# caiyuanhao1998/Open-DiffusionGS

Hardware: NVIDIA H100
Metric: denoise_steps_per_sec (higher is better)
Workload: dtype bf16

## Files before the change

### open-diffusiongs_b200/csrc/attention_sm90.cu

```cuda
#include "dgs_internal.h"
#include "dit_kernels.h"
#include "sm90_ptx.cuh"

namespace dgs {

using namespace ptx;

constexpr int ATT_BM = 128, ATT_BN = 128, ATT_HD = 64, ATT_KV_STAGES = 3, ATT_THREADS = WS_THREADS;
constexpr int ATT_Q_BYTES = ATT_BM * ATT_HD * 2;
constexpr int ATT_KV_BYTES = ATT_BN * ATT_HD * 2;
constexpr int ATT_SMEM_BYTES = ATT_Q_BYTES + 2 * ATT_KV_STAGES * ATT_KV_BYTES + 1024 + 256;

__global__ void __launch_bounds__(ATT_THREADS, 1)
attention_fwd_kernel(const __grid_constant__ CUtensorMap tm_qkv, __nv_bfloat16* __restrict__ out, float* __restrict__ lse2,
                     int Np, int N, int H) {
  extern __shared__ uint8_t smem_raw[];
  const uint32_t raw = smem_u32(smem_raw);
  uint8_t* smem = smem_raw + (((raw + 1023u) & ~1023u) - raw);
  uint8_t* sQ = smem;
  uint8_t* sK = sQ + ATT_Q_BYTES;
  uint8_t* sV = sK + ATT_KV_STAGES * ATT_KV_BYTES;
  uint64_t* q_full = reinterpret_cast<uint64_t*>(sV + ATT_KV_STAGES * ATT_KV_BYTES);
  uint64_t* k_full = q_full + 1;
  uint64_t* v_full = k_full + ATT_KV_STAGES;
  uint64_t* kv_empty = v_full + ATT_KV_STAGES;

  const int warp = threadIdx.x >> 5, lane = threadIdx.x & 31;
  const int q0 = blockIdx.x * ATT_BM, h = blockIdx.y, b = blockIdx.z;
  const int n_blocks = (N + ATT_BN - 1) / ATT_BN;
  const int D = H * ATT_HD;

  if (threadIdx.x == 0) {
    prefetch_tmap(&tm_qkv);
    mbar_init(q_full, 1);
    for (int s = 0; s < ATT_KV_STAGES; s++) { mbar_init(k_full + s, 1); mbar_init(v_full + s, 1); mbar_init(kv_empty + s, 8); }
    fence_barrier_init();
  }
  __syncthreads();
  griddep_launch_dependents();
  griddep_wait();

  if (warp >= 8) {
    ws_producer_regs();
    if (warp == 8 && lane == 0) {
      mbar_arrive_expect_tx(q_full, ATT_Q_BYTES);
      tma_load_3d(sQ, &tm_qkv, q_full, h * ATT_HD, q0, b);
      for (int j = 0; j < n_blocks; j++) {
        const int s = j % ATT_KV_STAGES;
        mbar_wait(kv_empty + s, ((uint32_t)(j / ATT_KV_STAGES) & 1) ^ 1);
        mbar_arrive_expect_tx(k_full + s, ATT_KV_BYTES);
        tma_load_3d(sK + s * ATT_KV_BYTES, &tm_qkv, k_full + s, D + h * ATT_HD, j * ATT_BN, b);
        mbar_arrive_expect_tx(v_full + s, ATT_KV_BYTES);
        tma_load_3d(sV + s * ATT_KV_BYTES, &tm_qkv, v_full + s, 2 * D + h * ATT_HD, j * ATT_BN, b);
      }
    }
    return;
  }

  ws_consumer_regs();
  const int wg = warp >> 2;
  const int quad_col = 2 * (lane & 3);
  const int r0 = wg * 64 + (warp & 3) * 16 + (lane >> 2);
  const float sl2 = 0.125f * 1.4426950408889634f;
  const uint64_t qdesc = wg_desc_sw128(smem_u32(sQ + wg * 8192), 16, 1024);
  float o[32];
#pragma unroll
  for (int i = 0; i < 32; i++) o[i] = 0.f;
  float m_run[2] = {-INFINITY, -INFINITY}, l_run[2] = {0.f, 0.f};
  mbar_wait(q_full, 0);
  for (int j = 0; j < n_blocks; j++) {
    const int s = j % ATT_KV_STAGES;
    const uint32_t use = (uint32_t)(j / ATT_KV_STAGES) & 1;
    float sc[64];
#pragma unroll
    for (int i = 0; i < 64; i++) sc[i] = 0.f;
    mbar_wait(k_full + s, use);
    {
      const uint64_t kdesc = wg_desc_sw128(smem_u32(sK + s * ATT_KV_BYTES), 16, 1024);
      wg_fence();
#pragma unroll
      for (int k = 0; k < ATT_HD / 16; k++) wgmma_m64n128_ss<0, 0>(sc, qdesc + (uint64_t)(2 * k), kdesc + (uint64_t)(2 * k));
      wg_commit();
      wg_wait<0>();
      wg_fence_regs(sc);
    }
    const int kv_valid = N - j * ATT_BN;
    if (kv_valid < ATT_BN) {
#pragma unroll
      for (int jj = 0; jj < 16; jj++)
#pragma unroll
        for (int e = 0; e < 4; e++)
          if (8 * jj + quad_col + (e & 1) >= kv_valid) sc[4 * jj + e] = -INFINITY;
    }
    float alpha[2], moff[2];
#pragma unroll
    for (int i = 0; i < 2; i++) {
      float mx = -INFINITY;
#pragma unroll
      for (int jj = 0; jj < 16; jj++) mx = fmaxf(mx, fmaxf(sc[4 * jj + 2 * i], sc[4 * jj + 2 * i + 1]));
      mx = fmaxf(mx, __shfl_xor_sync(0xffffffffu, mx, 1));
      mx = fmaxf(mx, __shfl_xor_sync(0xffffffffu, mx, 2));
      const float m_new = fmaxf(m_run[i], mx);
      alpha[i] = ex2_approx((m_run[i] - m_new) * sl2);
      m_run[i] = m_new;
      moff[i] = m_new * sl2;
    }
    uint32_t pa[8][4];
    float ls[2] = {0.f, 0.f};
#pragma unroll
    for (int kk = 0; kk < 8; kk++) {
#pragma unroll
      for (int q = 0; q < 4; q++) {
        const int idx = 8 * kk + 4 * (q >> 1) + 2 * (q & 1);
        const float p0 = ex2_approx(fmaf(sc[idx], sl2, -moff[q & 1]));
        const float p1 = ex2_approx(fmaf(sc[idx + 1], sl2, -moff[q & 1]));
        ls[q & 1] += p0 + p1;
        pa[kk][q] = pack2_bf16(p0, p1);
      }
    }
#pragma unroll
    for (int i = 0; i < 2; i++) l_run[i] = l_run[i] * alpha[i] + ls[i];
#pragma unroll
    for (int jj = 0; jj < 8; jj++) {
      o[4 * jj + 0] *= alpha[0]; o[4 * jj + 1] *= alpha[0];
      o[4 * jj + 2] *= alpha[1]; o[4 * jj + 3] *= alpha[1];
    }
    mbar_wait(v_full + s, use);
    {
      const uint64_t vdesc = wg_desc_sw128(smem_u32(sV + s * ATT_KV_BYTES), 8192, 1024);
      wg_fence();
#pragma unroll
      for (int kk = 0; kk < 8; kk++) wgmma_m64n64_rs<1>(o, pa[kk], vdesc + (uint64_t)(128 * kk));
      wg_commit();
      wg_wait<0>();
      wg_fence_regs(o);
    }
    __syncwarp();
    if (lane == 0) mbar_arrive(kv_empty + s);
  }
#pragma unroll
  for (int i = 0; i < 2; i++) {
    l_run[i] += __shfl_xor_sync(0xffffffffu, l_run[i], 1);
    l_run[i] += __shfl_xor_sync(0xffffffffu, l_run[i], 2);
  }
#pragma unroll
  for (int i = 0; i < 2; i++) {
    const int q = q0 + r0 + 8 * i;
    if (q >= N) continue;
    if (lse2 && (lane & 3) == 0) lse2[((size_t)b * H + h) * Np + q] = fmaf(m_run[i], sl2, log2f(l_run[i]));
    const float inv = 1.0f / l_run[i];
    __nv_bfloat16* dst = out + ((size_t)b * N + q) * D + h * ATT_HD + quad_col;
#pragma unroll
    for (int jj = 0; jj < 8; jj++)
      *reinterpret_cast<uint32_t*>(dst + 8 * jj) = pack2_bf16(o[4 * jj + 2 * i] * inv, o[4 * jj + 2 * i + 1] * inv);
  }
}

int attention_fwd(const void* qkv, void* out, float* lse2, int B, int N, int H, cudaStream_t st) {
  DGS_REQUIRE(B > 0 && N > 0 && H > 0, "attention: bad shape B=%d N=%d H=%d", B, N, H);
  const int D = H * ATT_HD;
  const int Np = attention_lse_stride(N);
  CUtensorMap tm_qkv;
  uint64_t dims[3] = {(uint64_t)(3 * D), (uint64_t)N, (uint64_t)B};
  uint64_t str[2] = {(uint64_t)(3 * D) * 2, (uint64_t)N * 3 * D * 2};
  uint32_t box[3] = {ATT_HD, ATT_BM, 1};
  int rc = make_tmap_bf16(&tm_qkv, qkv, 3, dims, str, box);
  if (rc) return rc;
  static bool configured = false;
  if (!configured) {
    DGS_CUDA_OK(cudaFuncSetAttribute(attention_fwd_kernel, cudaFuncAttributeMaxDynamicSharedMemorySize, ATT_SMEM_BYTES));
    configured = true;
  }
  dim3 grid(ceil_div(N, ATT_BM), H, B);
  DGS_CUDA_OK(launch_pdl(attention_fwd_kernel, grid, dim3(ATT_THREADS), ATT_SMEM_BYTES, st, tm_qkv,
                         reinterpret_cast<__nv_bfloat16*>(out), lse2, Np, N, H));
  DGS_POST_LAUNCH();
  return DGS_OK;
}

}
```

### open-diffusiongs_b200/csrc/sm90_ptx.cuh

```cuda
#pragma once
#include <cuda.h>
#include <cuda_bf16.h>
#include <cuda_runtime.h>

#include <cstdint>

namespace dgs {
namespace ptx {

__device__ __forceinline__ uint32_t smem_u32(const void* p) { return (uint32_t)__cvta_generic_to_shared(p); }

__device__ __forceinline__ void mbar_init(uint64_t* bar, uint32_t count) {
  asm volatile("mbarrier.init.shared::cta.b64 [%0], %1;" ::"r"(smem_u32(bar)), "r"(count) : "memory");
}
__device__ __forceinline__ void fence_barrier_init() { asm volatile("fence.mbarrier_init.release.cluster;" ::: "memory"); }
__device__ __forceinline__ void fence_proxy_async() { asm volatile("fence.proxy.async.shared::cta;" ::: "memory"); }
__device__ __forceinline__ void mbar_arrive_expect_tx(uint64_t* bar, uint32_t bytes) {
  asm volatile("mbarrier.arrive.expect_tx.shared::cta.b64 _, [%0], %1;" ::"r"(smem_u32(bar)), "r"(bytes) : "memory");
}
__device__ __forceinline__ void mbar_arrive(uint64_t* bar) {
  asm volatile("mbarrier.arrive.shared::cta.b64 _, [%0];" ::"r"(smem_u32(bar)) : "memory");
}
__device__ __forceinline__ bool mbar_try_wait(uint64_t* bar, uint32_t parity) {
  uint32_t ok;
  asm volatile(
      "{\n\t.reg .pred p;\n\t"
      "mbarrier.try_wait.parity.shared::cta.b64 p, [%1], %2;\n\t"
      "selp.b32 %0, 1, 0, p;\n\t}"
      : "=r"(ok)
      : "r"(smem_u32(bar)), "r"(parity)
      : "memory");
  return ok != 0;
}
__device__ __forceinline__ bool mbar_try_wait_hint(uint64_t* bar, uint32_t parity, uint32_t hint_ns) {
  uint32_t ok;
  asm volatile(
      "{\n\t.reg .pred p;\n\t"
      "mbarrier.try_wait.parity.shared::cta.b64 p, [%1], %2, %3;\n\t"
      "selp.b32 %0, 1, 0, p;\n\t}"
      : "=r"(ok)
      : "r"(smem_u32(bar)), "r"(parity), "r"(hint_ns)
      : "memory");
  return ok != 0;
}
#ifndef DGS_MBAR_TIMEOUT_SPINS
#define DGS_MBAR_TIMEOUT_SPINS 200000u
#endif
__device__ __forceinline__ void mbar_wait(uint64_t* bar, uint32_t parity) {
  if (mbar_try_wait(bar, parity)) return;
  uint32_t spins = 0;
  while (!mbar_try_wait_hint(bar, parity, 20000u)) {
    if (++spins > DGS_MBAR_TIMEOUT_SPINS) __trap();
  }
}

constexpr int WS_THREADS = 384;
__device__ __forceinline__ void ws_producer_regs() { asm volatile("setmaxnreg.dec.sync.aligned.u32 40;"); }
__device__ __forceinline__ void ws_consumer_regs() { asm volatile("setmaxnreg.inc.sync.aligned.u32 232;"); }

__device__ __forceinline__ void griddep_wait() { asm volatile("griddepcontrol.wait;" ::: "memory"); }
__device__ __forceinline__ void griddep_launch_dependents() { asm volatile("griddepcontrol.launch_dependents;" ::: "memory"); }

__device__ __forceinline__ void prefetch_tmap(const CUtensorMap* m) {
  asm volatile("prefetch.tensormap [%0];" ::"l"(reinterpret_cast<uint64_t>(m)) : "memory");
}
__device__ __forceinline__ void tma_load_2d(void* smem_dst, const CUtensorMap* m, uint64_t* bar, int c0, int c1) {
  asm volatile(
      "cp.async.bulk.tensor.2d.shared::cluster.global.mbarrier::complete_tx::bytes [%0], [%1, {%3, %4}], [%2];" ::"r"(
          smem_u32(smem_dst)),
      "l"(reinterpret_cast<uint64_t>(m)), "r"(smem_u32(bar)), "r"(c0), "r"(c1)
      : "memory");
}
__device__ __forceinline__ void tma_load_3d(void* smem_dst, const CUtensorMap* m, uint64_t* bar, int c0, int c1, int c2) {
  asm volatile(
      "cp.async.bulk.tensor.3d.shared::cluster.global.mbarrier::complete_tx::bytes [%0], [%1, {%3, %4, %5}], [%2];" ::"r"(
          smem_u32(smem_dst)),
      "l"(reinterpret_cast<uint64_t>(m)), "r"(smem_u32(bar)), "r"(c0), "r"(c1), "r"(c2)
      : "memory");
}
__device__ __forceinline__ void tma_store_2d(const CUtensorMap* m, const void* smem_src, int c0, int c1) {
  asm volatile("cp.async.bulk.tensor.2d.global.shared::cta.bulk_group [%0, {%2, %3}], [%1];" ::"l"(
                   reinterpret_cast<uint64_t>(m)),
               "r"(smem_u32(smem_src)), "r"(c0), "r"(c1)
               : "memory");
}
__device__ __forceinline__ void tma_reduce_add_2d(const CUtensorMap* m, const void* smem_src, int c0, int c1) {
  asm volatile("cp.reduce.async.bulk.tensor.2d.global.shared::cta.add.tile.bulk_group [%0, {%2, %3}], [%1];" ::"l"(
                   reinterpret_cast<uint64_t>(m)),
               "r"(smem_u32(smem_src)), "r"(c0), "r"(c1)
               : "memory");
}
__device__ __forceinline__ void bulk_commit() { asm volatile("cp.async.bulk.commit_group;" ::: "memory"); }
template <int N>
__device__ __forceinline__ void bulk_wait_read() { asm volatile("cp.async.bulk.wait_group.read %0;" ::"n"(N) : "memory"); }
template <int N>
__device__ __forceinline__ void bulk_wait() { asm volatile("cp.async.bulk.wait_group %0;" ::"n"(N) : "memory"); }
__device__ __forceinline__ void named_bar_sync(int id, int threads) {
  asm volatile("bar.sync %0, %1;" ::"r"(id), "r"(threads) : "memory");
}

__device__ __forceinline__ float ex2_approx(float x) {
  float y;
  asm("ex2.approx.ftz.f32 %0, %1;" : "=f"(y) : "f"(x));
  return y;
}
__device__ __forceinline__ uint32_t pack2_bf16(float a, float b) {
  __nv_bfloat162 v = __floats2bfloat162_rn(a, b);
  return *reinterpret_cast<uint32_t*>(&v);
}

__device__ __forceinline__ uint64_t wg_desc_sw128(uint32_t smem_addr, uint32_t lbo_bytes, uint32_t sbo_bytes) {
  uint64_t d = 0;
  d |= (uint64_t)((smem_addr & 0x3FFFFu) >> 4);
  d |= (uint64_t)((lbo_bytes >> 4) & 0x3FFFu) << 16;
  d |= (uint64_t)((sbo_bytes >> 4) & 0x3FFFu) << 32;
  d |= (uint64_t)1 << 62;
  return d;
}
__device__ __forceinline__ void wg_fence() { asm volatile("wgmma.fence.sync.aligned;" ::: "memory"); }
__device__ __forceinline__ void wg_commit() { asm volatile("wgmma.commit_group.sync.aligned;" ::: "memory"); }
template <int N>
__device__ __forceinline__ void wg_wait() { asm volatile("wgmma.wait_group.sync.aligned %0;" ::"n"(N) : "memory"); }
template <int R>
__device__ __forceinline__ void wg_fence_regs(float (&d)[R]) {
#pragma unroll
  for (int i = 0; i < R; i++) asm volatile("" : "+f"(d[i])::"memory");
}

template <int TA, int TB>
__device__ __forceinline__ void wgmma_m64n256_ss(float (&d)[128], uint64_t da, uint64_t db) {
  asm volatile(
      "wgmma.mma_async.sync.aligned.m64n256k16.f32.bf16.bf16 "
      "{%0, %1, %2, %3, %4, %5, %6, %7, %8, %9, %10, %11, %12, %13, %14, %15, %16, %17, %18, %19, %20, %21, %22, %23, %24, %25, %26, %27, %28, %29, %30, %31, %32, %33, %34, %35, %36, %37, %38, %39, %40, %41, %42, %43, %44, %45, %46, %47, %48, %49, %50, %51, %52, %53, %54, %55, %56, %57, %58, %59, %60, %61, %62, %63, %64, %65, %66, %67, %68, %69, %70, %71, %72, %73, %74, %75, %76, %77, %78, %79, %80, %81, %82, %83, %84, %85, %86, %87, %88, %89, %90, %91, %92, %93, %94, %95, %96, %97, %98, %99, %100, %101, %102, %103, %104, %105, %106, %107, %108, %109, %110, %111, %112, %113, %114, %115, %116, %117, %118, %119, %120, %121, %122, %123, %124, %125, %126, %127}, %128, %129, 1, 1, 1, %130, %131;"
      : "+f"(d[0]), "+f"(d[1]), "+f"(d[2]), "+f"(d[3]), "+f"(d[4]), "+f"(d[5]), "+f"(d[6]), "+f"(d[7]), "+f"(d[8]), "+f"(d[9]), "+f"(d[10]), "+f"(d[11]), "+f"(d[12]), "+f"(d[13]), "+f"(d[14]), "+f"(d[15]), "+f"(d[16]), "+f"(d[17]), "+f"(d[18]), "+f"(d[19]), "+f"(d[20]), "+f"(d[21]), "+f"(d[22]), "+f"(d[23]), "+f"(d[24]), "+f"(d[25]), "+f"(d[26]), "+f"(d[27]), "+f"(d[28]), "+f"(d[29]), "+f"(d[30]), "+f"(d[31]), "+f"(d[32]), "+f"(d[33]), "+f"(d[34]), "+f"(d[35]), "+f"(d[36]), "+f"(d[37]), "+f"(d[38]), "+f"(d[39]), "+f"(d[40]), "+f"(d[41]), "+f"(d[42]), "+f"(d[43]), "+f"(d[44]), "+f"(d[45]), "+f"(d[46]), "+f"(d[47]), "+f"(d[48]), "+f"(d[49]), "+f"(d[50]), "+f"(d[51]), "+f"(d[52]), "+f"(d[53]), "+f"(d[54]), "+f"(d[55]), "+f"(d[56]), "+f"(d[57]), "+f"(d[58]), "+f"(d[59]), "+f"(d[60]), "+f"(d[61]), "+f"(d[62]), "+f"(d[63]), "+f"(d[64]), "+f"(d[65]), "+f"(d[66]), "+f"(d[67]), "+f"(d[68]), "+f"(d[69]), "+f"(d[70]), "+f"(d[71]), "+f"(d[72]), "+f"(d[73]), "+f"(d[74]), "+f"(d[75]), "+f"(d[76]), "+f"(d[77]), "+f"(d[78]), "+f"(d[79]), "+f"(d[80]), "+f"(d[81]), "+f"(d[82]), "+f"(d[83]), "+f"(d[84]), "+f"(d[85]), "+f"(d[86]), "+f"(d[87]), "+f"(d[88]), "+f"(d[89]), "+f"(d[90]), "+f"(d[91]), "+f"(d[92]), "+f"(d[93]), "+f"(d[94]), "+f"(d[95]), "+f"(d[96]), "+f"(d[97]), "+f"(d[98]), "+f"(d[99]), "+f"(d[100]), "+f"(d[101]), "+f"(d[102]), "+f"(d[103]), "+f"(d[104]), "+f"(d[105]), "+f"(d[106]), "+f"(d[107]), "+f"(d[108]), "+f"(d[109]), "+f"(d[110]), "+f"(d[111]), "+f"(d[112]), "+f"(d[113]), "+f"(d[114]), "+f"(d[115]), "+f"(d[116]), "+f"(d[117]), "+f"(d[118]), "+f"(d[119]), "+f"(d[120]), "+f"(d[121]), "+f"(d[122]), "+f"(d[123]), "+f"(d[124]), "+f"(d[125]), "+f"(d[126]), "+f"(d[127])
      : "l"(da), "l"(db), "n"(TA), "n"(TB));
}
template <int TA, int TB>
__device__ __forceinline__ void wgmma_m64n128_ss(float (&d)[64], uint64_t da, uint64_t db) {
  asm volatile(
      "wgmma.mma_async.sync.aligned.m64n128k16.f32.bf16.bf16 "
      "{%0, %1, %2, %3, %4, %5, %6, %7, %8, %9, %10, %11, %12, %13, %14, %15, %16, %17, %18, %19, %20, %21, %22, %23, %24, %25, %26, %27, %28, %29, %30, %31, %32, %33, %34, %35, %36, %37, %38, %39, %40, %41, %42, %43, %44, %45, %46, %47, %48, %49, %50, %51, %52, %53, %54, %55, %56, %57, %58, %59, %60, %61, %62, %63}, %64, %65, 1, 1, 1, %66, %67;"
      : "+f"(d[0]), "+f"(d[1]), "+f"(d[2]), "+f"(d[3]), "+f"(d[4]), "+f"(d[5]), "+f"(d[6]), "+f"(d[7]), "+f"(d[8]), "+f"(d[9]), "+f"(d[10]), "+f"(d[11]), "+f"(d[12]), "+f"(d[13]), "+f"(d[14]), "+f"(d[15]), "+f"(d[16]), "+f"(d[17]), "+f"(d[18]), "+f"(d[19]), "+f"(d[20]), "+f"(d[21]), "+f"(d[22]), "+f"(d[23]), "+f"(d[24]), "+f"(d[25]), "+f"(d[26]), "+f"(d[27]), "+f"(d[28]), "+f"(d[29]), "+f"(d[30]), "+f"(d[31]), "+f"(d[32]), "+f"(d[33]), "+f"(d[34]), "+f"(d[35]), "+f"(d[36]), "+f"(d[37]), "+f"(d[38]), "+f"(d[39]), "+f"(d[40]), "+f"(d[41]), "+f"(d[42]), "+f"(d[43]), "+f"(d[44]), "+f"(d[45]), "+f"(d[46]), "+f"(d[47]), "+f"(d[48]), "+f"(d[49]), "+f"(d[50]), "+f"(d[51]), "+f"(d[52]), "+f"(d[53]), "+f"(d[54]), "+f"(d[55]), "+f"(d[56]), "+f"(d[57]), "+f"(d[58]), "+f"(d[59]), "+f"(d[60]), "+f"(d[61]), "+f"(d[62]), "+f"(d[63])
      : "l"(da), "l"(db), "n"(TA), "n"(TB));
}
template <int TA, int TB>
__device__ __forceinline__ void wgmma_m64n64_ss(float (&d)[32], uint64_t da, uint64_t db) {
  asm volatile(
      "wgmma.mma_async.sync.aligned.m64n64k16.f32.bf16.bf16 "
      "{%0, %1, %2, %3, %4, %5, %6, %7, %8, %9, %10, %11, %12, %13, %14, %15, %16, %17, %18, %19, %20, %21, %22, %23, %24, %25, %26, %27, %28, %29, %30, %31}, %32, %33, 1, 1, 1, %34, %35;"
      : "+f"(d[0]), "+f"(d[1]), "+f"(d[2]), "+f"(d[3]), "+f"(d[4]), "+f"(d[5]), "+f"(d[6]), "+f"(d[7]), "+f"(d[8]), "+f"(d[9]), "+f"(d[10]), "+f"(d[11]), "+f"(d[12]), "+f"(d[13]), "+f"(d[14]), "+f"(d[15]), "+f"(d[16]), "+f"(d[17]), "+f"(d[18]), "+f"(d[19]), "+f"(d[20]), "+f"(d[21]), "+f"(d[22]), "+f"(d[23]), "+f"(d[24]), "+f"(d[25]), "+f"(d[26]), "+f"(d[27]), "+f"(d[28]), "+f"(d[29]), "+f"(d[30]), "+f"(d[31])
      : "l"(da), "l"(db), "n"(TA), "n"(TB));
}
template <int TB>
__device__ __forceinline__ void wgmma_m64n64_rs(float (&d)[32], const uint32_t (&a)[4], uint64_t db) {
  asm volatile(
      "wgmma.mma_async.sync.aligned.m64n64k16.f32.bf16.bf16 "
      "{%0, %1, %2, %3, %4, %5, %6, %7, %8, %9, %10, %11, %12, %13, %14, %15, %16, %17, %18, %19, %20, %21, %22, %23, %24, %25, %26, %27, %28, %29, %30, %31}, {%32, %33, %34, %35}, %36, 1, 1, 1, %37;"
      : "+f"(d[0]), "+f"(d[1]), "+f"(d[2]), "+f"(d[3]), "+f"(d[4]), "+f"(d[5]), "+f"(d[6]), "+f"(d[7]), "+f"(d[8]), "+f"(d[9]), "+f"(d[10]), "+f"(d[11]), "+f"(d[12]), "+f"(d[13]), "+f"(d[14]), "+f"(d[15]), "+f"(d[16]), "+f"(d[17]), "+f"(d[18]), "+f"(d[19]), "+f"(d[20]), "+f"(d[21]), "+f"(d[22]), "+f"(d[23]), "+f"(d[24]), "+f"(d[25]), "+f"(d[26]), "+f"(d[27]), "+f"(d[28]), "+f"(d[29]), "+f"(d[30]), "+f"(d[31])
      : "r"(a[0]), "r"(a[1]), "r"(a[2]), "r"(a[3]), "l"(db), "n"(TB));
}

}

int make_tmap(CUtensorMap* out, CUtensorMapDataType dtype, const void* base, int rank, const uint64_t* dims,
              const uint64_t* strides_bytes, const uint32_t* box);
inline int make_tmap_bf16(CUtensorMap* out, const void* base, int rank, const uint64_t* dims, const uint64_t* strides_bytes,
                          const uint32_t* box) {
  return make_tmap(out, CU_TENSOR_MAP_DATA_TYPE_BFLOAT16, base, rank, dims, strides_bytes, box);
}

}
```

Before: 64.12.

## Software-pipeline attention QK/PV with warpgroup ping-pong and narrow tail block

Restructures the flash-attention consumer loop so that the QK^T wgmma of block j is issued together with the PV wgmma of block j-1, and the two consumer warpgroups take turns on the tensor cores through named barriers so one group's softmax overlaps the other's MMAs. K and V stages get separate empty barriers so K buffers are released earlier, and the stage count grows from 3 to 4. A final partial key block of 16 or fewer keys uses an m64n16 wgmma instead of a full 128-wide one. This adds register pressure (sc plus pa live across the MMAs) and more complex barrier phasing, which risks spills or ordering bugs.

```diff
diff --git a/open-diffusiongs_b200/csrc/attention_sm90.cu b/open-diffusiongs_b200/csrc/attention_sm90.cu
--- a/open-diffusiongs_b200/csrc/attention_sm90.cu
+++ b/open-diffusiongs_b200/csrc/attention_sm90.cu
@@ -2,14 +2,95 @@
 #include "dit_kernels.h"
 #include "sm90_ptx.cuh"
 
+#include <type_traits>
+
 namespace dgs {
 
 using namespace ptx;
 
-constexpr int ATT_BM = 128, ATT_BN = 128, ATT_HD = 64, ATT_KV_STAGES = 3, ATT_THREADS = WS_THREADS;
+constexpr int ATT_BM = 128, ATT_BN = 128, ATT_HD = 64, ATT_KV_STAGES = 4, ATT_THREADS = WS_THREADS;
+constexpr int ATT_TAIL_BN = 16;
 constexpr int ATT_Q_BYTES = ATT_BM * ATT_HD * 2;
 constexpr int ATT_KV_BYTES = ATT_BN * ATT_HD * 2;
 constexpr int ATT_SMEM_BYTES = ATT_Q_BYTES + 2 * ATT_KV_STAGES * ATT_KV_BYTES + 1024 + 256;
+static_assert(8 * (1 + 4 * ATT_KV_STAGES) <= 256, "attention: mbarriers exceed their shared-memory slot");
+static_assert(ATT_SMEM_BYTES <= 227 * 1024, "attention: shared memory over the sm_90 per-block limit");
+
+template <int NJ>
+__device__ __forceinline__ void att_qk(float (&sc)[4 * NJ], uint64_t qdesc, uint64_t kdesc, int zero_d) {
+  if constexpr (NJ == 16) {
+    wgmma_m64n128_ss_z<0, 0>(sc, qdesc, kdesc, zero_d);
+#pragma unroll
+    for (int k = 1; k < ATT_HD / 16; k++) wgmma_m64n128_ss<0, 0>(sc, qdesc + (uint64_t)(2 * k), kdesc + (uint64_t)(2 * k));
+  } else {
+    static_assert(NJ == 2, "att_qk: 128 or 16 keys");
+    wgmma_m64n16_ss<0, 0, 0>(sc, qdesc, kdesc);
+#pragma unroll
+    for (int k = 1; k < ATT_HD / 16; k++) wgmma_m64n16_ss<0, 0>(sc, qdesc + (uint64_t)(2 * k), kdesc + (uint64_t)(2 * k));
+  }
+}
+
+template <int NK>
+__device__ __forceinline__ void att_pv(float (&o)[32], const uint32_t (&pa)[8][4], uint64_t vdesc) {
+#pragma unroll
+  for (int kk = 0; kk < NK; kk++) wgmma_m64n64_rs<1>(o, pa[kk], vdesc + (uint64_t)(128 * kk));
+}
+
+template <int NJ>
+__device__ __forceinline__ void att_softmax(float (&sc)[4 * NJ], int kv_valid, int quad_col, float (&m_run)[2], float (&l_run)[2],
+                                            float (&alpha)[2]) {
+  constexpr float sl2 = 0.125f * 1.4426950408889634f;
+  if (kv_valid < 8 * NJ) {
+#pragma unroll
+    for (int jj = 0; jj < NJ; jj++)
+#pragma unroll
+      for (int e = 0; e < 4; e++)
+        if (8 * jj + quad_col + (e & 1) >= kv_valid) sc[4 * jj + e] = -INFINITY;
+  }
+  float mx[2];
+#pragma unroll
+  for (int i = 0; i < 2; i++) {
+    mx[i] = -INFINITY;
+#pragma unroll
+    for (int jj = 0; jj < NJ; jj++) mx[i] = fmaxf(mx[i], fmaxf(sc[4 * jj + 2 * i], sc[4 * jj + 2 * i + 1]));
+    mx[i] = fmaxf(mx[i], __shfl_xor_sync(0xffffffffu, mx[i], 1));
+    mx[i] = fmaxf(mx[i], __shfl_xor_sync(0xffffffffu, mx[i], 2));
+  }
+  float moff[2];
+#pragma unroll
+  for (int i = 0; i < 2; i++) {
+    const float m_new = fmaxf(m_run[i], mx[i]);
+    alpha[i] = ex2_approx((m_run[i] - m_new) * sl2);
+    m_run[i] = m_new;
+    moff[i] = m_new * sl2;
+  }
+  float ls[2] = {0.f, 0.f};
+#pragma unroll
+  for (int kk = 0; kk < NJ / 2; kk++) {
+#pragma unroll
+    for (int q = 0; q < 4; q++) {
+      const int idx = 8 * kk + 4 * (q >> 1) + 2 * (q & 1);
+      const float p0 = ex2_approx(fmaf(sc[idx], sl2, -moff[q & 1]));
+      const float p1 = ex2_approx(fmaf(sc[idx + 1], sl2, -moff[q & 1]));
+      ls[q & 1] += p0 + p1;
+      sc[idx] = p0;
+      sc[idx + 1] = p1;
+    }
+  }
+#pragma unroll
+  for (int i = 0; i < 2; i++) l_run[i] = l_run[i] * alpha[i] + ls[i];
+}
+
+template <int NK>
+__device__ __forceinline__ void att_pack(const float (&sc)[8 * NK], uint32_t (&pa)[8][4]) {
+#pragma unroll
+  for (int kk = 0; kk < NK; kk++)
+#pragma unroll
+    for (int q = 0; q < 4; q++) {
+      const int idx = 8 * kk + 4 * (q >> 1) + 2 * (q & 1);
+      pa[kk][q] = pack2_bf16(sc[idx], sc[idx + 1]);
+    }
+}
 
 __global__ void __launch_bounds__(ATT_THREADS, 1)
 attention_fwd_kernel(const __grid_constant__ CUtensorMap tm_qkv, __nv_bfloat16* __restrict__ out, float* __restrict__ lse2,
@@ -23,7 +104,8 @@
   uint64_t* q_full = reinterpret_cast<uint64_t*>(sV + ATT_KV_STAGES * ATT_KV_BYTES);
   uint64_t* k_full = q_full + 1;
   uint64_t* v_full = k_full + ATT_KV_STAGES;
-  uint64_t* kv_empty = v_full + ATT_KV_STAGES;
+  uint64_t* k_empty = v_full + ATT_KV_STAGES;
+  uint64_t* v_empty = k_empty + ATT_KV_STAGES;
 
   const int warp = threadIdx.x >> 5, lane = threadIdx.x & 31;
   const int q0 = blockIdx.x * ATT_BM, h = blockIdx.y, b = blockIdx.z;
@@ -33,7 +115,12 @@
   if (threadIdx.x == 0) {
     prefetch_tmap(&tm_qkv);
     mbar_init(q_full, 1);
-    for (int s = 0; s < ATT_KV_STAGES; s++) { mbar_init(k_full + s, 1); mbar_init(v_full + s, 1); mbar_init(kv_empty + s, 8); }
+    for (int s = 0; s < ATT_KV_STAGES; s++) {
+      mbar_init(k_full + s, 1);
+      mbar_init(v_full + s, 1);
+      mbar_init(k_empty + s, 8);
+      mbar_init(v_empty + s, 8);
+    }
     fence_barrier_init();
   }
   __syncthreads();
@@ -47,9 +134,11 @@
       tma_load_3d(sQ, &tm_qkv, q_full, h * ATT_HD, q0, b);
       for (int j = 0; j < n_blocks; j++) {
         const int s = j % ATT_KV_STAGES;
-        mbar_wait(kv_empty + s, ((uint32_t)(j / ATT_KV_STAGES) & 1) ^ 1);
+        const uint32_t free_phase = ((uint32_t)(j / ATT_KV_STAGES) & 1) ^ 1;
+        mbar_wait(k_empty + s, free_phase);
         mbar_arrive_expect_tx(k_full + s, ATT_KV_BYTES);
         tma_load_3d(sK + s * ATT_KV_BYTES, &tm_qkv, k_full + s, D + h * ATT_HD, j * ATT_BN, b);
+        mbar_wait(v_empty + s, free_phase);
         mbar_arrive_expect_tx(v_full + s, ATT_KV_BYTES);
         tma_load_3d(sV + s * ATT_KV_BYTES, &tm_qkv, v_full + s, 2 * D + h * ATT_HD, j * ATT_BN, b);
       }
@@ -63,80 +152,92 @@
   const int r0 = wg * 64 + (warp & 3) * 16 + (lane >> 2);
   const float sl2 = 0.125f * 1.4426950408889634f;
   const uint64_t qdesc = wg_desc_sw128(smem_u32(sQ + wg * 8192), 16, 1024);
-  float o[32];
+  const bool narrow_tail = N - (n_blocks - 1) * ATT_BN <= ATT_TAIL_BN;
+  const int zero_s = n_blocks > 0;
+  auto kdesc = [&](int s) { return wg_desc_sw128(smem_u32(sK + s * ATT_KV_BYTES), 16, 1024); };
+  auto vdesc = [&](int s) { return wg_desc_sw128(smem_u32(sV + s * ATT_KV_BYTES), 8192, 1024); };
+  auto release = [&](uint64_t* bar) {
+    __syncwarp();
+    if (lane == 0) mbar_arrive(bar);
+  };
+  auto turn_wait = [&]() { named_bar_sync(1 + wg, 256); };
+  auto turn_pass = [&]() { named_bar_arrive(2 - wg, 256); };
+  if (wg == 1) turn_pass();
+
+  float o[32], sc[64];
 #pragma unroll
   for (int i = 0; i < 32; i++) o[i] = 0.f;
-  float m_run[2] = {-INFINITY, -INFINITY}, l_run[2] = {0.f, 0.f};
-  mbar_wait(q_full, 0);
-  for (int j = 0; j < n_blocks; j++) {
-    const int s = j % ATT_KV_STAGES;
-    const uint32_t use = (uint32_t)(j / ATT_KV_STAGES) & 1;
-    float sc[64];
-#pragma unroll
-    for (int i = 0; i < 64; i++) sc[i] = 0.f;
-    mbar_wait(k_full + s, use);
-    {
-      const uint64_t kdesc = wg_desc_sw128(smem_u32(sK + s * ATT_KV_BYTES), 16, 1024);
-      wg_fence();
-#pragma unroll
-      for (int k = 0; k < ATT_HD / 16; k++) wgmma_m64n128_ss<0, 0>(sc, qdesc + (uint64_t)(2 * k), kdesc + (uint64_t)(2 * k));
-      wg_commit();
-      wg_wait<0>();
-      wg_fence_regs(sc);
-    }
-    const int kv_valid = N - j * ATT_BN;
-    if (kv_valid < ATT_BN) {
-#pragma unroll
-      for (int jj = 0; jj < 16; jj++)
-#pragma unroll
-        for (int e = 0; e < 4; e++)
-          if (8 * jj + quad_col + (e & 1) >= kv_valid) sc[4 * jj + e] = -INFINITY;
-    }
-    float alpha[2], moff[2];
-#pragma unroll
-    for (int i = 0; i < 2; i++) {
-      float mx = -INFINITY;
-#pragma unroll
-      for (int jj = 0; jj < 16; jj++) mx = fmaxf(mx, fmaxf(sc[4 * jj + 2 * i], sc[4 * jj + 2 * i + 1]));
-      mx = fmaxf(mx, __shfl_xor_sync(0xffffffffu, mx, 1));
-      mx = fmaxf(mx, __shfl_xor_sync(0xffffffffu, mx, 2));
-      const float m_new = fmaxf(m_run[i], mx);
-      alpha[i] = ex2_approx((m_run[i] - m_new) * sl2);
-      m_run[i] = m_new;
-      moff[i] = m_new * sl2;
-    }
-    uint32_t pa[8][4];
-    float ls[2] = {0.f, 0.f};
-#pragma unroll
-    for (int kk = 0; kk < 8; kk++) {
-#pragma unroll
-      for (int q = 0; q < 4; q++) {
-        const int idx = 8 * kk + 4 * (q >> 1) + 2 * (q & 1);
-        const float p0 = ex2_approx(fmaf(sc[idx], sl2, -moff[q & 1]));
-        const float p1 = ex2_approx(fmaf(sc[idx + 1], sl2, -moff[q & 1]));
-        ls[q & 1] += p0 + p1;
-        pa[kk][q] = pack2_bf16(p0, p1);
-      }
-    }
-#pragma unroll
-    for (int i = 0; i < 2; i++) l_run[i] = l_run[i] * alpha[i] + ls[i];
+#pragma unroll
+  for (int i = 0; i < 64; i++) sc[i] = 0.f;
+  uint32_t pa[8][4];
+  float m_run[2] = {-INFINITY, -INFINITY}, l_run[2] = {0.f, 0.f}, alpha[2] = {1.f, 1.f};
+  auto rescale_o = [&]() {
 #pragma unroll
     for (int jj = 0; jj < 8; jj++) {
       o[4 * jj + 0] *= alpha[0]; o[4 * jj + 1] *= alpha[0];
       o[4 * jj + 2] *= alpha[1]; o[4 * jj + 3] *= alpha[1];
     }
-    mbar_wait(v_full + s, use);
-    {
-      const uint64_t vdesc = wg_desc_sw128(smem_u32(sV + s * ATT_KV_BYTES), 8192, 1024);
-      wg_fence();
-#pragma unroll
-      for (int kk = 0; kk < 8; kk++) wgmma_m64n64_rs<1>(o, pa[kk], vdesc + (uint64_t)(128 * kk));
-      wg_commit();
+  };
+  auto key_block = [&](int j, auto& s_acc, auto first_block) {
+    constexpr int NJ = sizeof(s_acc) / sizeof(float) / 4;
+    constexpr bool FIRST = decltype(first_block)::value;
+    const int s = j % ATT_KV_STAGES, sp = (j + ATT_KV_STAGES - 1) % ATT_KV_STAGES;
+    mbar_wait(k_full + s, (uint32_t)(j / ATT_KV_STAGES) & 1);
+    if constexpr (!FIRST) {
+      mbar_wait(v_full + sp, (uint32_t)((j - 1) / ATT_KV_STAGES) & 1);
       wg_wait<0>();
       wg_fence_regs(o);
-    }
-    __syncwarp();
-    if (lane == 0) mbar_arrive(kv_empty + s);
+      if (j >= 2) release(v_empty + (j - 2) % ATT_KV_STAGES);
+      rescale_o();
+      att_pack<8>(sc, pa);
+    }
+    turn_wait();
+    wg_fence();
+    att_qk<NJ>(s_acc, qdesc, kdesc(s), zero_s);
+    wg_commit();
+    if constexpr (!FIRST) {
+      att_pv<8>(o, pa, vdesc(sp));
+      wg_commit();
+      turn_pass();
+      wg_wait<1>();
+    } else {
+      turn_pass();
+      wg_wait<0>();
+    }
+    wg_fence_regs(s_acc);
+    release(k_empty + s);
+    att_softmax<NJ>(s_acc, N - j * ATT_BN, quad_col, m_run, l_run, alpha);
+  };
+  mbar_wait(q_full, 0);
+  const int n_full = narrow_tail ? n_blocks - 1 : n_blocks;
+  float st[8];
+#pragma unroll
+  for (int i = 0; i < 8; i++) st[i] = 0.f;
+  if (n_full > 0) key_block(0, sc, std::true_type{});
+  for (int j = 1; j < n_full; j++) key_block(j, sc, std::false_type{});
+  if (narrow_tail) {
+    if (n_full > 0) key_block(n_full, st, std::false_type{});
+    else key_block(0, st, std::true_type{});
+  }
+  {
+    const int s = (n_blocks - 1) % ATT_KV_STAGES;
+    mbar_wait(v_full + s, (uint32_t)((n_blocks - 1) / ATT_KV_STAGES) & 1);
+    wg_wait<0>();
+    wg_fence_regs(o);
+    rescale_o();
+    turn_wait();
+    wg_fence();
+    if (narrow_tail) {
+      att_pack<1>(st, pa);
+      att_pv<1>(o, pa, vdesc(s));
+    } else {
+      att_pack<8>(sc, pa);
+      att_pv<8>(o, pa, vdesc(s));
+    }
+    wg_commit();
+    if (wg == 0) turn_pass();
+    wg_wait<0>();
+    wg_fence_regs(o);
   }
 #pragma unroll
   for (int i = 0; i < 2; i++) {
diff --git a/open-diffusiongs_b200/csrc/sm90_ptx.cuh b/open-diffusiongs_b200/csrc/sm90_ptx.cuh
--- a/open-diffusiongs_b200/csrc/sm90_ptx.cuh
+++ b/open-diffusiongs_b200/csrc/sm90_ptx.cuh
@@ -98,6 +98,9 @@
 __device__ __forceinline__ void named_bar_sync(int id, int threads) {
   asm volatile("bar.sync %0, %1;" ::"r"(id), "r"(threads) : "memory");
 }
+__device__ __forceinline__ void named_bar_arrive(int id, int threads) {
+  asm volatile("bar.arrive %0, %1;" ::"r"(id), "r"(threads) : "memory");
+}
 
 __device__ __forceinline__ float ex2_approx(float x) {
   float y;
@@ -144,6 +147,23 @@
       : "l"(da), "l"(db), "n"(TA), "n"(TB));
 }
 template <int TA, int TB>
+__device__ __forceinline__ void wgmma_m64n128_ss_z(float (&d)[64], uint64_t da, uint64_t db, int zero_d) {
+  asm volatile(
+      "{\n\t.reg .pred p;\n\tsetp.eq.s32 p, %68, 0;\n\t"
+      "wgmma.mma_async.sync.aligned.m64n128k16.f32.bf16.bf16 "
+      "{%0, %1, %2, %3, %4, %5, %6, %7, %8, %9, %10, %11, %12, %13, %14, %15, %16, %17, %18, %19, %20, %21, %22, %23, %24, %25, %26, %27, %28, %29, %30, %31, %32, %33, %34, %35, %36, %37, %38, %39, %40, %41, %42, %43, %44, %45, %46, %47, %48, %49, %50, %51, %52, %53, %54, %55, %56, %57, %58, %59, %60, %61, %62, %63}, %64, %65, p, 1, 1, %66, %67;\n\t}"
+      : "+f"(d[0]), "+f"(d[1]), "+f"(d[2]), "+f"(d[3]), "+f"(d[4]), "+f"(d[5]), "+f"(d[6]), "+f"(d[7]), "+f"(d[8]), "+f"(d[9]), "+f"(d[10]), "+f"(d[11]), "+f"(d[12]), "+f"(d[13]), "+f"(d[14]), "+f"(d[15]), "+f"(d[16]), "+f"(d[17]), "+f"(d[18]), "+f"(d[19]), "+f"(d[20]), "+f"(d[21]), "+f"(d[22]), "+f"(d[23]), "+f"(d[24]), "+f"(d[25]), "+f"(d[26]), "+f"(d[27]), "+f"(d[28]), "+f"(d[29]), "+f"(d[30]), "+f"(d[31]), "+f"(d[32]), "+f"(d[33]), "+f"(d[34]), "+f"(d[35]), "+f"(d[36]), "+f"(d[37]), "+f"(d[38]), "+f"(d[39]), "+f"(d[40]), "+f"(d[41]), "+f"(d[42]), "+f"(d[43]), "+f"(d[44]), "+f"(d[45]), "+f"(d[46]), "+f"(d[47]), "+f"(d[48]), "+f"(d[49]), "+f"(d[50]), "+f"(d[51]), "+f"(d[52]), "+f"(d[53]), "+f"(d[54]), "+f"(d[55]), "+f"(d[56]), "+f"(d[57]), "+f"(d[58]), "+f"(d[59]), "+f"(d[60]), "+f"(d[61]), "+f"(d[62]), "+f"(d[63])
+      : "l"(da), "l"(db), "n"(TA), "n"(TB), "r"(zero_d));
+}
+template <int TA, int TB, int SD = 1>
+__device__ __forceinline__ void wgmma_m64n16_ss(float (&d)[8], uint64_t da, uint64_t db) {
+  asm volatile(
+      "wgmma.mma_async.sync.aligned.m64n16k16.f32.bf16.bf16 "
+      "{%0, %1, %2, %3, %4, %5, %6, %7}, %8, %9, %12, 1, 1, %10, %11;"
+      : "+f"(d[0]), "+f"(d[1]), "+f"(d[2]), "+f"(d[3]), "+f"(d[4]), "+f"(d[5]), "+f"(d[6]), "+f"(d[7])
+      : "l"(da), "l"(db), "n"(TA), "n"(TB), "n"(SD));
+}
+template <int TA, int TB>
 __device__ __forceinline__ void wgmma_m64n64_ss(float (&d)[32], uint64_t da, uint64_t db) {
   asm volatile(
       "wgmma.mma_async.sync.aligned.m64n64k16.f32.bf16.bf16 "
```

Result: no change. 64.93, median of 6 (+1.3%).
